# elcritch/figdraw

Hardware: AMD Instinct MI355X
Metric: Mpixels/s composited @3840x2160, 300 SDF rects+shadows; % HBM roofline (higher is better)
Workload: dtype f32 (blur taps: u8 x f16 -> f32 MFMA); 1 GPU; S300@4K: renderlist_100 scene at 3840x2160, 300 shadowed SDF rects + full-frame and 360x240 2-pass Gaussian backdrop blur(18) (BASELINE.json configs[2]); draws=707, phases=3, blur_nodes=2, fragments=41088819, parallelism=single GPU, frames_in_flight_per_gpu=4, walk_pool_threads=7, walk_pool_threads_default=7

## Files before the change

### figdraw_amd/context.py

```python
from __future__ import annotations

import ctypes as C
import os
import subprocess
from typing import Optional

import numpy as np

from . import scene as S

_HERE = os.path.dirname(os.path.abspath(__file__))
LIB_PATH = os.path.join(_HERE, "libfigdraw_hip.so")
_lib = None

_F4 = C.c_float * 4
_F2 = C.c_float * 2
_COL4 = S.CColor * 4


class FigdrawHipError(RuntimeError):
    def __init__(self, code: int, msg: str):
        super().__init__(f"[{code}] {msg}")
        self.code = code

# ... 90 lines not shown
    if hasattr(L, "fdh_put_glyph_outlines"):
        L.fdh_put_glyph_outlines.argtypes = [vp, vp, C.c_int, C.c_uint32, vp]
        L.fdh_glyph_batch_stats.argtypes = [vp, C.POINTER(GlyphBatchStats)]
        L.fdh_sizeof_glyph_outline.argtypes = []
    if hasattr(L, "fdh_put_glyph_outline_cubic"):
        L.fdh_put_glyph_outline_cubic.argtypes = [vp, C.c_int64, C.c_int, C.c_int, vp, C.c_int, C.c_uint32, C.c_int * 4]
    if hasattr(L, "fdh_put_glyph_coverage_batch"):
        L.fdh_put_glyph_coverage_batch.argtypes = [vp, vp, C.c_int, C.c_uint32, vp]
        L.fdh_glyph_coverage_batch_stats.argtypes = [vp, C.POINTER(GlyphBatchStats)]
    if hasattr(L, "fdh_put_glyph_outlines_cubic"):
        L.fdh_put_glyph_outlines_cubic.argtypes = [vp, vp, C.c_int, C.c_uint32, vp]
        L.fdh_put_glyph_coverage_batch_cubic.argtypes = [vp, vp, C.c_int, C.c_uint32, vp]
    L.fdh_read_pixels.argtypes = [vp, C.c_int, C.c_int, C.c_int, C.c_int, vp]
    L.fdh_debug_read_surface.argtypes = [vp, C.c_int, vp]
    L.fdh_scene_retain.argtypes = [vp, vp, C.c_float, C.c_float, C.c_int, _F4]
    L.fdh_scene_update_nodes.argtypes = [vp, C.c_int, C.c_int, C.c_int, vp, vp]
    L.fdh_scene_replace_root.argtypes = [vp, C.c_int, C.c_int, vp, C.c_int, vp]
    L.fdh_scene_insert_root.argtypes = [vp, C.c_int, C.c_int, vp, C.c_int, vp]
    L.fdh_scene_render.argtypes = [vp]
    L.fdh_scene_stats.argtypes = [vp, C.POINTER(C.c_int64), C.POINTER(C.c_int64)]
    L.fdh_debug_record_digest.argtypes = [vp, C.POINTER(C.c_uint64)]
    L.fdh_debug_verify_upload.argtypes = [vp, C.POINTER(C.c_uint32)]
    L.fdh_debug_bin_digest.argtypes = [vp, C.POINTER(C.c_uint64)]
    L.fdh_debug_staging_store_bytes.argtypes = [C.c_int, C.POINTER(C.c_int64)]
    L.fdh_last_upload_bytes.argtypes = [vp, C.POINTER(C.c_int64)]
    L.fdh_record_begin.argtypes = [vp]
    L.fdh_record_json.argtypes = [vp]
    L.fdh_record_json.restype = C.c_char_p
    L.fdh_frame_device_ptr.argtypes = [vp, C.POINTER(vp), C.POINTER(C.c_int), C.POINTER(C.c_int), C.POINTER(C.c_int64)]
    L.fdh_sync.argtypes = [vp]
    L.fdh_flush.argtypes = [vp]
    L.fdh_set_ui_scale.argtypes = [vp, C.c_float]
    L.fdh_render_frame.argtypes = [vp, vp, C.c_float, C.c_float, C.c_int, _F4]
    L.fdh_set_stripe.argtypes = [vp, C.c_int, C.c_int]
    L.fdh_set_blur_route.argtypes = [vp, C.c_int]
    L.fdh_set_cull.argtypes = [vp, C.c_int]
    L.fdh_culled_draws.argtypes = [vp, C.POINTER(C.c_int64)]
    L.fdh_set_walk_threads.argtypes = [vp, C.c_int]
    L.fdh_debug_host_times.argtypes = [vp, C.POINTER(C.c_int64)]
    L.fdh_walk_stats.argtypes = [vp, C.POINTER(C.c_int), C.POINTER(C.c_int64)]
    L.fdh_stripe_rows.argtypes = [C.c_int, C.c_int, C.c_int, C.POINTER(C.c_int), C.POINTER(C.c_int)]
    L.fdh_comm_unique_id.argtypes = [C.c_char_p]
    L.fdh_comm_init.argtypes = [vp, C.c_char_p, C.c_int, C.c_int]
    L.fdh_comm_destroy.argtypes = [vp]
    L.fdh_comm_share.argtypes = [vp, vp]
    L.fdh_gather_stripes.argtypes = [vp, C.c_int, vp]
# ... 363 lines not shown
    def scene_render(self):
        self._ck(self.L.fdh_scene_render(self.h))

    def scene_stats(self):
        a, b = C.c_int64(), C.c_int64()
        self._ck(self.L.fdh_scene_stats(self.h, C.byref(a), C.byref(b)))
        return a.value, b.value

    def last_upload_bytes(self) -> int:
        out = C.c_int64()
        self._ck(self.L.fdh_last_upload_bytes(self.h, C.byref(out)))
        return out.value

    def verify_upload(self):
        out = (C.c_uint32 * 24)()
        self._ck(self.L.fdh_debug_verify_upload(self.h, out))
        return list(out)

    def bin_digest(self):
        out = (C.c_uint64 * 8)()
        self._ck(self.L.fdh_debug_bin_digest(self.h, out))
        return list(out)[:5]

    def record_digest(self) -> int:
        out = C.c_uint64()
        self._ck(self.L.fdh_debug_record_digest(self.h, C.byref(out)))
        return out.value

    def replay_calls(self, calls):
        for call in calls:
            name, args = call[0], call[1:]
            if name == "begin_frame":
                self.begin_frame(self.W, self.H, *args)
            else:
                getattr(self, name)(*args)

    def set_stripe(self, y0: int, y1: int):
        self._ck(self.L.fdh_set_stripe(self.h, int(y0), int(y1)))

    def set_cull(self, mode: int):
        self._ck(self.L.fdh_set_cull(self.h, int(mode)))

    def set_walk_threads(self, n: int):
        self._ck(self.L.fdh_set_walk_threads(self.h, int(n)))

    def host_times(self):
# ... 218 lines not shown
```

### figdraw_amd/csrc/fdh_capi.cpp

```cpp
#include <string>

#include "fdh_context.h"
#include "fdh_damage.h"
#include "../../include/figdraw_hip_damage.h"
#include "../../include/figdraw_hip_pick.h"
#include "../../include/figdraw_hip_readback.h"
#include "../../include/figdraw_hip_stream.h"
#include "../../include/figdraw_hip_exact.h"
#include "../../include_glyphs/figdraw_hip_glyphs.h"
#include "../../include_glyphs/figdraw_hip_coverage.h"
#include "../../include_glyphs/figdraw_hip_cubic.h"

using fdh::Context;

namespace {
thread_local std::string g_last_error;

template <typename F>
int guard(F&& f) {
  try {
    f();
    return FDH_OK;
  } catch (const fdh::Error& e) {
    g_last_error = e.what();
// ... 11 lines not shown
  return reinterpret_cast<Context*>(c);
}
}

extern "C" {

const char* fdh_last_error(void) { return g_last_error.c_str(); }
#if FDH_STATS
extern "C++" { namespace fdh { void debug_counters(unsigned long long out[128], bool reset); void debug_wave_times(unsigned long long* out); } }
__attribute__((visibility("default"))) int fdh_debug_wave_times(unsigned long long* out) { fdh::debug_wave_times(out); return 0; }
__attribute__((visibility("default"))) int fdh_debug_counters(unsigned long long out[128], int reset) { fdh::debug_counters(out, reset != 0); return 0; }
#endif
int fdh_saturated_core(const float rect[4], const float rx[4], const float ry[4], int mode, float factor, float spread,
                       const float shape[2], float aa, int out_px[4]) {
  return guard([&] { fdh::saturated_core_of(rect, rx, ry, mode, factor, spread, shape, aa, out_px); });
}
__attribute__((visibility("default"))) int fdh_saturated_core_union(const float rect[4], const float rx[4], const float ry[4], int mode, float factor, float spread,
                             const float shape[2], float aa, int push, int out_px[12], int* n_out) {
  return guard([&] {
    if (!out_px || !n_out) throw fdh::Error(FDH_ERR_INVALID, "fdh_saturated_core_union: null pointer");
    *n_out = fdh::saturated_core_union_of(rect, rx, ry, mode, factor, spread, shape, aa, push, out_px);
  });
}
int fdh_blur_weight_fragments(float blur_radius, int vertical, float* dense, uint16_t* frag_bits, int* reach, int* k_steps) {
  return guard([&] {
    if (!dense || !frag_bits || !reach || !k_steps) throw fdh::Error(FDH_ERR_INVALID, "fdh_blur_weight_fragments: null pointer");
    fdh::blur_weight_fragments(blur_radius, vertical != 0, dense, frag_bits, reach, k_steps);
  });
}
const char* fdh_version(void) { return "figdraw_hip 0.1.0 (gfx950)"; }
int fdh_sizeof_fig(void) { return (int)sizeof(FdhFig); }
int fdh_sizeof_glyph(void) { return (int)sizeof(FdhGlyph); }
int fdh_sizeof_draw_op(void) { return (int)sizeof(FdhDrawOp); }
int fdh_sizeof_text_rect(void) { return (int)sizeof(FdhTextRect); }

int fdh_create(FdhContext** out, int atlas_size, float pixel_scale, int device, uint32_t flags) {
  return guard([&] {
    if (!out) throw fdh::Error(FDH_ERR_INVALID, "fdh_create: null out pointer");
    *out = nullptr;
    *out = reinterpret_cast<FdhContext*>(new Context(atlas_size, pixel_scale, device, flags));
  });
}
int fdh_destroy(FdhContext* c) { return guard([&] { delete C(c); }); }
int fdh_set_stream(FdhContext* c, void* s) { return guard([&] { C(c)->set_stream(s); }); }

int fdh_begin_frame(FdhContext* c, int w, int h, int clear, const float rgba[4]) {
// ... 323 lines not shown
```

### figdraw_amd/csrc/fdh_context.h

```cpp
#pragma once
#include <hip/hip_runtime.h>

#include <algorithm>
#include <atomic>
#include <chrono>
#include <condition_variable>
#include <cstdint>
#include <cstdlib>
#include <cstring>
#include <exception>
#include <memory>
#include <mutex>
#include <stdexcept>
#include <string>
#include <thread>
#include <unordered_map>
#include <vector>

#include "../../include/figdraw_hip.h"
#include "../../include/figdraw_hip_pick.h"
#include "../../include/figdraw_hip_readback.h"
#include "../../include/figdraw_hip_stream.h"
#include "fdh_kernels.h"
#include "fdh_plain.h"
// ... 122 lines not shown
  void reset_atlas(int minimum_size) { sync(); atlas_.reset(minimum_size, stream_); }
  int atlas_size() const { return atlas_.size(); }
  int64_t atlas_packed_area() const { return atlas_.packed_area(); }

  void read_pixels(int x, int y, int w, int h, uint8_t* out);
  void frame_device_ptr(void** p, int* w, int* h, int64_t* pitch_bytes);
  void debug_read_surface(int which, uint8_t* out);
  void record_begin();
  const char* record_json();
  void sync();
  void set_stream(void* s);

  void set_ui_scale(float s) { ui_scale_ = s; }
  float ui_scale() const { return ui_scale_; }
  void render_frame(const FdhScene* scene, float fw, float fh, bool clear, const float rgba[4]);
  void scene_retain(const FdhScene* scene, float fw, float fh, bool clear, const float rgba[4]) { retained_.retain(scene, fw, fh, clear, rgba); scene_render(); }
  void scene_update_nodes(int layer, int first, int count, const FdhFig* nodes, const FdhScene* side) { retained_.update_nodes(layer, first, count, nodes, side); }
  void scene_replace_root(int layer, int slot, const FdhFig* subtree, int n, const FdhScene* side, bool insert) { retained_.replace_root(layer, slot, subtree, n, side, insert); }
  void scene_render();
  void scene_stats(int64_t* walked, int64_t* reused) const { retained_.stats(walked, reused); }
  int64_t uploaded_bytes() { drain(); return uploaded_bytes_; }
  void debug_verify_upload(uint32_t out[24]);
  void debug_bin_digest(uint64_t out[8]);
  uint64_t record_digest();

  void comm_init(const uint8_t id[FDH_COMM_ID_BYTES], int rank, int world);
  void comm_share(Context* owner);
  void comm_destroy();
  void gather_stripes(int dst_rank, void* dst_image);
  void gather_frames(int dst_rank, void* const* dst_images);
  int comm_world() const { return comm_ ? comm_world_ : 1; }

  void set_stripe(int y0, int y1) {
    drain();
    if (damage_.on && y1 > y0) throw Error(FDH_ERR_INVALID, "fdh_set_stripe: damage tracking is on (fdh_set_damage_tracking: not under row stripes)");
    if (readback_.on && y1 > y0) throw Error(FDH_ERR_INVALID, "fdh_set_stripe: damage readback is on (fdh_set_damage_readback: not under row stripes)");
    stripe_y0_ = y0; stripe_y1_ = y1;
  }
  void set_damage_tracking(bool on);
  void damage_bins(uint8_t* mask, int cap, int* bins_x, int* bins_y, int* n_damaged, bool changed_only);
  void set_damage_readback(bool on);
  void read_damage(const FdhDamageTile** tiles, const uint8_t** pixels, int* n_tiles, int* frame_w, int* frame_h, int* full);
  void read_damage_into(uint8_t* image, int64_t pitch_bytes, int w, int h, int* n_tiles);
  void read_damage_coded(const FdhCodedTile** tiles, const uint8_t** payload, int* n_tiles, int64_t* payload_bytes, int* frame_w, int* frame_h, int* full);
  void set_damage_exact(bool on);
  void damage_exact_stats(int* n_pending, int* n_changed, int* fresh);
// ... 227 lines not shown
```

### figdraw_amd/csrc/fdh_debug.cpp

```cpp
#include "fdh_context.h"

#include <cstring>

namespace fdh {

uint64_t Context::record_digest() {
  drain();
  uint64_t h = 1469598103934665603ull;
  auto mix = [&](const void* p, size_t n) { const uint8_t* b = static_cast<const uint8_t*>(p); for (size_t i = 0; i < n; i++) { h ^= b[i]; h *= 1099511628211ull; } };
  const uint64_t n = n_total_;
  mix(&n, sizeof n);
  uint32_t ext_base = 0;
  for (const Piece& p : pieces_) {
    const Lane& L = lane(p.lane);
    for (uint32_t i = 0; i < p.n; i++) {
      DrawRec r = L.recs[p.first + i];
      record_host_form(r);
      if (r.op_mode & F_GENERAL) r.ext = r.ext - p.ext_first + ext_base;
      mix(&r, sizeof r);
    }
    ext_base += p.n_ext;
  }
  for (const Piece& p : pieces_) { const Lane& L = lane(p.lane); for (uint32_t i = 0; i < p.n; i++) mix(&L.bins[p.first + i].box, sizeof(BBox)); }
  for (const Piece& p : pieces_) { const Lane& L = lane(p.lane); for (uint32_t i = 0; i < p.n_ext; i++) mix(&L.exts[p.ext_first + i], sizeof(QuadExt)); }
// ... 85 lines not shown
  std::vector<uint2> lists(np * nb * stride);
  FDH_HIP(hipMemcpy(counts.data(), J.counts, counts.size() * 4, hipMemcpyDeviceToHost));
  FDH_HIP(hipMemcpy(lists.data(), J.lists, lists.size() * sizeof(uint2), hipMemcpyDeviceToHost));
  uint64_t h = 1469598103934665603ull;
  auto mix = [&](uint32_t v) { for (int k = 0; k < 4; k++) { h ^= (v >> (8 * k)) & 255u; h *= 1099511628211ull; } };
  for (size_t p = 0; p < np; p++) {
    const Phase& ph = J.phases[p];
    const bool whole = p == 0;
    for (int by = 0; by < J.bins_y; by++)
      for (int bx = 0; bx < J.bins_x; bx++) {
        if (!whole && (bx < ph.bin_x0 || bx >= ph.bin_x1 || by < ph.bin_y0 || by >= ph.bin_y1)) continue;
        const size_t b = p * nb + (size_t)by * J.bins_x + bx;
        const uint32_t c = counts[b];
        mix(c);
        out[1] += c;
        if (c == 0) out[2]++;
        if (c > stride) { out[4]++; continue; }
        for (uint32_t e = 0; e < c; e++) { const uint2 v = lists[b * stride + e]; mix(v.x); mix(v.y); if (v.x == 0) out[3]++; }
      }
  }
  out[0] = h;
}

void Context::debug_read_surface(int which, uint8_t* out) {
  need_device("debug_read_surface");
  drain();
  if (which == 4) {
    FDH_HIP(hipSetDevice(device_));
    FDH_HIP(hipStreamSynchronize(stream_));
    FDH_HIP(hipMemcpy(out, atlas_.level0(), (size_t)atlas_.size() * atlas_.size() * 4, hipMemcpyDeviceToHost));
    return;
  }
  const uint32_t* src = which == 0 ? fb_ : which == 1 ? blur_tmp_ : which == 2 ? backdrop_ : which == 3 ? dbg_snap_ : nullptr;
  if (!src) throw Error(FDH_ERR_INVALID, "debug_read_surface: no such surface (or no frame yet)");
  FDH_HIP(hipSetDevice(device_));
  FDH_HIP(hipStreamSynchronize(stream_));
  FDH_HIP(hipMemcpy(out, src, (size_t)W_ * H_ * 4, hipMemcpyDeviceToHost));
}

}
```

### figdraw_amd/csrc/fdh_record.cpp

```cpp
#include <algorithm>
#include <cmath>
#include <cstdio>
#include <cstring>

#include "fdh_context.h"
#include "fdh_host.h"

namespace fdh {

void Recorder::shrink_to_ink(const AtlasEntry& e, bool use_alpha, int level_t) {
  static const bool enabled = [] { const char* v = std::getenv("FDH_INK_BOUNDS"); return !v || std::atoi(v) != 0; }();
  if (!enabled || !e.has_ink || level_t < 0 || lane_->recs.empty()) return;
  DrawRec& r = lane_->recs.back();
  BBox& b = lane_->bins.back().box;
  if ((r.op_mode & F_GENERAL) || b.x1 <= b.x0 || b.y1 <= b.y0) return;
  const InkBox ib = (use_alpha ? e.ink_a : e.ink_rgb)[std::min(level_t / 16, kInkLevels - 1)];
  if (ib.x1 <= ib.x0 || ib.y1 <= ib.y0) { b = BBox{0, 0, 0, 0}; r.bx0 = r.by0 = r.bx1 = r.by1 = 0; return; }
  const double S = (double)cx_->atlas_.size();
  auto range = [&](double ua, double ut, double o, double inv, double lo_t, double hi_t, int& p0, int& p1) {
    const double A = (ut - ua) * inv * S, B = ua * S - 0.5 - A * o;
    if (!(std::fabs(A) > 1e-12)) return;
    double c0 = ((lo_t - 3.0) - B) / A, c1 = ((hi_t + 2.0) - B) / A;
    if (c0 > c1) std::swap(c0, c1);
    if (!(c0 > -1.0e6 && c1 < 1.0e6)) return;
// ... 118 lines not shown
  flags |= BR_HAS_CORE | (rot ? BR_GENERAL : 0u);
  if (op == OP_DRAW && (mode == 9u || mode == 11u || mode == 12u)) {
    flags |= BR_CORE_REMOVED;
    if (!rot && (om & F_SOLID) && fill_mode == 0u && mode != 11u) flags |= ((mode == 9u ? 3u : 4u) + ell) << LE_PATH_SHIFT;
  } else {
    if (op == OP_DRAW && (om & F_SOLID) && fill_mode == 0u && mode != 17u) {
      flags |= LE_PLAIN;
      const uint32_t code = mode == 3u ? 1u : mode == 7u ? 2u : 0u;
      if (code && !rot) flags |= (code + ell) << LE_PATH_SHIFT;
    }
    if (op == OP_DRAW && mode == 3u) {
      uint32_t a = r.col[0] & r.col[1] & r.col[2] & r.col[3];
      if (fill_mode != 0u) a &= r.mid & r.stop;
      if ((a >> 24) == 255u) flags |= LE_OPAQUE;
    }
  }
  return flags;
}
static inline bool colour_as_floats(uint32_t om) {
  const uint32_t mode = om & 255u;
  const bool atlas_mode = mode == 0u || (mode >= 13u && mode <= 16u);
  return !(((om & F_GENERAL) && !(om & F_EDGE32)) || atlas_mode || mode >= 18u || ((om >> 12) & 15u) != OP_DRAW || !(om & F_SOLID));
}
void record_host_form(DrawRec& r) {
  if (colour_as_floats(r.op_mode)) r.col[1] = r.col[2] = r.col[3] = r.col[0];
}

void Recorder::link_share(uint32_t idx) {
  if ((int)idx <= phase_floor_) return;
  const DrawRec& b = lane_->recs[idx];
  BinRec& pa = lane_->bins[idx - 1];
  const uint32_t code = (pa.flags >> LE_PATH_SHIFT) & 15u;
  if (code == 0u) return;
  const DrawRec& r = lane_->recs[idx - 1];
  const uint32_t om = r.op_mode, mode = om & 255u;
  if (mode == 7u) return;
  const uint32_t omb = b.op_mode, modeb = omb & 255u;
  const bool simple_b = ((omb >> 12) & 15u) == OP_DRAW && !(omb & F_GENERAL) && (omb & F_SOLID) && ((omb >> 9) & 7u) == 0u &&
                        (modeb == 3u || modeb == 9u || modeb == 12u) && ((omb ^ om) & F_ELLIP) == 0u;
  if (simple_b && std::memcmp(&r.ox, &b.ox, 6 * sizeof(float)) == 0 && std::memcmp(r.r, b.r, sizeof r.r) == 0 &&
      std::memcmp(&r.bx0, &b.bx0, 4 * sizeof(int16_t)) == 0 && r.aa == b.aa) {
    const float sax = mode == 9u ? r.p0 : r.p2, say = mode == 9u ? r.p1 : r.p3, sbx = modeb == 9u ? b.p0 : b.p2, sby = modeb == 9u ? b.p1 : b.p3;
    if (sax == sbx && say == sby) pa.flags |= LE_SHARE;
  }
}

void Recorder::commit_bins(uint32_t idx) {
  DrawRec& r = lane_->recs[idx];
// ... 114 lines not shown
  const uint32_t mode = r.op_mode & 255u, op = (r.op_mode >> 12) & 15u;
  const uint32_t fill_mode = (r.op_mode >> 9) & 7u;
  if (!(op == OP_DRAW || op == OP_MASK_PUSH) || !(r.aa > 0.0f)) return false;
  double e;
  if (op == OP_MASK_PUSH || mode == FDH_SDF_CLIP_AA || mode == FDH_SDF_BACKDROP_BLUR) e = 0.5 / r.aa;
  else if (mode == FDH_SDF_DROP_SHADOW) e = std::max(0.0, -(double)(fill_mode == 0u ? r.f1 : 0.0f));
  else if (mode == FDH_SDF_ANNULAR || mode == FDH_SDF_ANNULAR_AA) e = std::max(0.0, (double)r.f0) + 0.5 / r.aa;
  else if (mode == FDH_SDF_INSET_SHADOW && op == OP_DRAW) {
    const double sigma = std::max(0.5 * (double)r.f0, 0.5);
    e = std::max(0.0, 3.7 * sigma + (double)(fill_mode == 0u ? r.f1 : 0.0f));
  } else return false;
  const bool inset = mode == FDH_SDF_INSET_SHADOW;
  const double qhx = r.p0, qhy = r.p1, bx = inset ? qhx : (double)r.p2, by = inset ? qhy : (double)r.p3;
  if (!(qhx > 0.0 && qhy > 0.0 && bx > 0.0 && by > 0.0)) return false;
  double crx[4], cry[4];
  for (int k = 0; k < 4; k++) {
    const double sel = r.r[k];
    if (!(r.op_mode & F_ELLIP)) { crx[k] = cry[k] = std::max(sel, 0.0); continue; }
    if (sel < 0.0) { crx[k] = cry[k] = -sel - 1.0; continue; }
    const double pv = std::floor(sel + 0.5), hi = std::floor(pv / 4096.0);
    crx[k] = (pv - 4096.0 * hi) * bx / 4095.0;
    cry[k] = hi * by / 4095.0;
  }
  enum { TR = 0, BR = 1, TL = 2, BL = 3 };
  LocalRect &H = out[1], &V = out[2];
  H.xl = -(bx - e); H.xr = bx - e;
  V.yb = -(by - e); V.yt = by - e;
  if (!(r.op_mode & F_ELLIP)) {
    const double k = 0.2929;
    auto rr = [&](int i) { return std::max(crx[i] - e, 0.0); };
    const double mr = std::max(rr(TR), rr(BR)), ml = std::max(rr(TL), rr(BL)), mt = std::max(rr(TR), rr(TL)), mb = std::max(rr(BR), rr(BL));
    out[0].xr = (bx - e) - k * mr;
    out[0].xl = -(bx - e) + k * ml;
    out[0].yt = (by - e) - k * mt;
    out[0].yb = -(by - e) + k * mb;
    H.yt = (by - e) - mt; H.yb = -(by - e) + mb;
    V.xr = (bx - e) - mr; V.xl = -(bx - e) + ml;
  } else {
    H.yt = std::min(by - e, by - std::max(cry[TR], cry[TL])); H.yb = -std::min(by - e, by - std::max(cry[BR], cry[BL]));
    V.xr = std::min(bx - e, bx - std::max(crx[TR], crx[BR])); V.xl = -std::min(bx - e, bx - std::max(crx[TL], crx[BL]));
    const double ah = std::max(H.xr - H.xl, 0.0) * std::max(H.yt - H.yb, 0.0), av = std::max(V.xr - V.xl, 0.0) * std::max(V.yt - V.yb, 0.0);
    out[0] = ah >= av ? H : V;
  }
  if (inset)
    for (int k = 0; k < 3; k++) { out[k].xl += r.p2; out[k].xr += r.p2; out[k].yb -= r.p3; out[k].yt -= r.p3; }
  return true;
}
static bool core_pixels(const DrawRec& r, float w_px, float h_px, const LocalRect& c, int16_t px[4]) {
  if (!c.ok()) return false;
  const double qhx = r.p0, qhy = r.p1;
#ifndef FDH_CORE_SLACK
#define FDH_CORE_SLACK (1.0 / 16.0)
#endif
  const double slack = FDH_CORE_SLACK;
  const double cxl = r.ox + w_px * (c.xl / (2.0 * qhx) + 0.5) + slack, cxr = r.ox + w_px * (c.xr / (2.0 * qhx) + 0.5) - slack;
  const double cyt = r.oy + h_px * (0.5 - c.yt / (2.0 * qhy)) + slack, cyb = r.oy + h_px * (0.5 - c.yb / (2.0 * qhy)) - slack;
  double ix0 = std::ceil(cxl - 0.5), ix1 = std::floor(cxr - 0.5) + 1.0, iy0 = std::ceil(cyt - 0.5), iy1 = std::floor(cyb - 0.5) + 1.0;
  ix0 = std::max(ix0, (double)r.ox); ix1 = std::min(ix1, (double)r.ox + w_px);
  iy0 = std::max(iy0, (double)r.oy); iy1 = std::min(iy1, (double)r.oy + h_px);
  auto c16 = [](double v) { return (int16_t)std::min(std::max(v, -32768.0), 32767.0); };
  if (!(ix1 > ix0 && iy1 > iy0)) return false;
  px[0] = c16(ix0); px[1] = c16(iy0); px[2] = c16(ix1); px[3] = c16(iy1);
  return true;
}
static bool core_union_on() {
  static const bool enabled = [] { const char* v = std::getenv("FDH_CORE_UNION"); return !v || std::atoi(v) != 0; }();
// ... 89 lines not shown
  const float* py = q.py;
  BBox b = q.b;
  bands_ = CoreBands{};
  const bool cullable = ((r.op_mode >> 12) & 15u) == OP_DRAW && culling();
  const float fields[] = {r.p0, r.p1, r.p2, r.p3, r.f0, r.f1, r.r[0], r.r[1], r.r[2], r.r[3], r.aa, r.aux, r.aux2};
  bool params_finite = true;
  for (const float v : fields) params_finite = params_finite && std::isfinite(v);
  if (!q.finite || !params_finite) {
    if (cullable) { FDH_CULLED(); return false; }
    r.bx0 = r.by0 = r.bx1 = r.by1 = 0; push_rec(b); return true;
  }
  if (cullable && !bbox_visible(b)) { FDH_CULLED(); return false; }
  r.bx0 = b.x0; r.by0 = b.y0; r.bx1 = b.x1; r.by1 = b.y1;
  const bool aligned = px[3] == px[0] && px[2] == px[1] && py[3] == py[2] && py[0] == py[1] && px[1] > px[0] && py[0] > py[3];
  const bool bezier = (r.op_mode & 255u) >= 18u && (r.op_mode & 255u) <= 20u;
  if (aligned) {
    r.ox = px[3];
    r.oy = py[3];
    r.inv_w = 1.0f / (px[1] - px[0]);
    r.inv_h = 1.0f / (py[0] - py[3]);
    r.kx = 2.0f * r.p0 * r.inv_w;
    r.ky = 2.0f * r.p1 * r.inv_h;
    if (!bezier) bands_ = set_saturated_core(r, px[1] - px[0], py[0] - py[3]);
  }
  if (!aligned || bezier) {
    QuadExt& q = *lane_->exts.slot();
    std::memset(static_cast<void*>(&q), 0, sizeof q);
    static const int TRI[2][3] = {{3, 0, 1}, {2, 3, 1}};
    const uint32_t mode = r.op_mode & 255u;
    const bool atlas_mode = mode == 0u || (mode >= 13u && mode <= 16u);
    const float uax = atlas_mode ? r.r[0] : 0.0f, uay = atlas_mode ? r.r[1] : 0.0f, utx = atlas_mode ? r.r[2] : 1.0f, uty = atlas_mode ? r.r[3] : 1.0f;
    const float vu[4] = {uax, utx, utx, uax}, vv[4] = {uty, uty, uay, uay};
    bool edge32 = true;
    const long long xm = 2LL * cx_->W_ + 129, ym = 2LL * cx_->H_ + 129;
    for (int t = 0; t < 2; t++) {
      long long X[3], Y[3];
      for (int k = 0; k < 3; k++) { X[k] = 2 * (long long)px[TRI[t][k]]; Y[k] = 2 * (long long)py[TRI[t][k]]; }
      long long area2 = (X[1] - X[0]) * (Y[2] - Y[0]) - (Y[1] - Y[0]) * (X[2] - X[0]);
      const long long sgn = area2 >= 0 ? 1 : -1;
      for (int k = 0; k < 3; k++) {
        const int i0 = (k + 1) % 3, i1 = (k + 2) % 3;
        long long A = -(Y[i1] - Y[i0]) * sgn, B = (X[i1] - X[i0]) * sgn;
        long long C = -(B * Y[i0]) - (A * X[i0]);
        q.e[t][k].a = (int32_t)A; q.e[t][k].b = (int32_t)B; q.e[t][k].c = C;
        {
          const long long aa = A < 0 ? -A : A, ab = B < 0 ? -B : B, ac = C < 0 ? -(C + 1) : C;
// ... 610 lines not shown
```

### figdraw_amd/csrc/fdh_types.h

```cpp
#pragma once
#include <stdint.h>

#ifndef FDH_MX_LO
#define FDH_MX_LO 0
#endif

namespace fdh {

constexpr int kTile = 8;
constexpr int kTileW = 4 * kTile;
constexpr int kTileH = kTile;
constexpr int kWavesPerWg = 4;
constexpr int kWgW = kTileW;
constexpr int kWgH = kTileH * kWavesPerWg;
constexpr int kBin = 64;
constexpr int kWgsPerBin = (kBin / kWgW) * (kBin / kWgH);
constexpr int kMaskDepth = 16;
constexpr int kDeepMinDefault = 24;
constexpr int kDeepMinInFlight = 40;
constexpr int kDeepStripMinDefault = 16;
constexpr int kMaxMips = 14;
constexpr int kMaxBlurTaps = 36;

enum : uint32_t { OP_DRAW = 0, OP_MASK_PUSH = 1, OP_MASK_POP = 2, OP_RMASK_BEGIN = 3, OP_RMASK_END = 4 };
// ... 6 lines not shown
constexpr uint32_t F_TEXEL_1TO1 = 1u << 20;
constexpr uint32_t F_EDGE32 = 1u << 21;

struct alignas(16) DrawRec {
  uint32_t op_mode;
  uint32_t ext;
  float ox, oy;
  float inv_w, inv_h;
  float p0, p1;
  float p2, p3;
  float f0, f1;
  float r[4];
  uint32_t col[4];
  uint32_t mid, stop;
  float aa;
  float aux;
  float aux2;
  int16_t bx0, by0, bx1, by1;
  int16_t ix0, iy0, ix1, iy1;
  float kx, ky;
  uint32_t _pad;
};
static_assert(sizeof(DrawRec) == 128, "DrawRec must be 128 bytes");

struct alignas(16) QuadExt {
  struct Edge { int32_t a, b; int64_t c; };
  Edge e[2][3];
  float inv_sum[2];
  uint32_t own;
  float fw_u[2], fw_v[2];
  float lod[2];
  float _pad[3];
  float core[4];
  float lm[2][6];
};
static_assert(sizeof(QuadExt) == 208 && offsetof(QuadExt, core) == 144 && offsetof(QuadExt, lm) == 160, "QuadExt: 208 bytes, core at 144, lm at 160");

struct alignas(8) BBox { int16_t x0, y0, x1, y1; };

struct alignas(8) BinRec { BBox box; int16_t ix0, iy0, ix1, iy1; uint32_t flags; uint32_t grow; uint16_t hy0, hy1, vx0, vx1; };
static_assert(sizeof(BinRec) == 32, "BinRec must be 32 bytes");
constexpr uint32_t BR_HAS_CORE = 1u, BR_CORE_REMOVED = 2u;
constexpr uint32_t BR_GENERAL = 4u;
constexpr uint32_t BR_CURVE = 8u;
constexpr uint32_t BR_BOX_EXACT = 16u;
constexpr uint32_t LE_PLAIN = 1u << 31;
// ... 33 lines not shown
```

### figdraw_amd/csrc/k_composite.hip

```cpp
#include "fdh_device.h"
#include "fdh_shade.h"
#include "fdh_damage.h"

#ifndef FDH_TU
#define FDH_TU 0
#endif

namespace fdh {

__device__ __forceinline__ void order_bins_wave(const uint32_t* __restrict__ counts, int* __restrict__ order, int nx, int nb, uint32_t* offs, int lane, int cls,
                                                int deep_min = 0, uint32_t* __restrict__ deep_out = nullptr) {
#pragma unroll
  for (int k = 0; k < 4; k++) offs[lane + 64 * k] = 0;
  __builtin_amdgcn_wave_barrier();
  constexpr int kU = 8;
  const int nc = (nb - cls + 7) >> 3;
  for (int i0 = lane; i0 < nc; i0 += 64 * kU) {
    uint32_t c[kU];
#pragma unroll
    for (int k = 0; k < kU; k++) c[k] = i0 + 64 * k < nc ? counts[cls + 8 * (i0 + 64 * k)] : 0xffffffffu;
#pragma unroll
    for (int k = 0; k < kU; k++) if (c[k] != 0xffffffffu) atomicAdd(&offs[255u - min(c[k], 255u)], 1u);
  }
  __builtin_amdgcn_wave_barrier();
// ... 9 lines not shown
    __builtin_amdgcn_wave_barrier();
    offs[4 * lane] = base; offs[4 * lane + 1] = base + a; offs[4 * lane + 2] = base + a + b; offs[4 * lane + 3] = base + a + b + c2;
  }
  __builtin_amdgcn_wave_barrier();
  if (deep_out != nullptr && lane == 0) {
    const int m = min(max(deep_min, 1), 255);
    __hip_atomic_store(deep_out + cls, offs[256 - m], __ATOMIC_RELAXED, __HIP_MEMORY_SCOPE_SYSTEM);
  }
  __builtin_amdgcn_wave_barrier();
  for (int i0 = lane; i0 < nc; i0 += 64 * kU) {
    uint32_t c[kU];
#pragma unroll
    for (int k = 0; k < kU; k++) c[k] = i0 + 64 * k < nc ? counts[cls + 8 * (i0 + 64 * k)] : 0xffffffffu;
#pragma unroll
    for (int k = 0; k < kU; k++)
      if (c[k] != 0xffffffffu) {
        const int i = cls + 8 * (i0 + 64 * k), row = i / nx;
        order[8 * (int)atomicAdd(&offs[255u - min(c[k], 255u)], 1u) + cls] = (row << 16) | (i - row * nx);
      }
  }
}

struct Corner { float rx, ry; bool same; };
__device__ __forceinline__ Corner pick_corner(bool ellip, float px, float py, float bx, float by, float r0, float r1, float r2, float r3) {
  const float sel = (px > 0.0f) ? ((py > 0.0f) ? r0 : r1) : ((py > 0.0f) ? r2 : r3);
  Corner c;
  if (!ellip) { c.rx = sel; c.ry = sel; c.same = true; return c; }
  const float pv = __builtin_floorf(sel + 0.5f);
  const float hi = __builtin_floorf(pv * (1.0f / 4096.0f));
  float rx = (pv - 4096.0f * hi) * bx * (1.0f / 4095.0f);
  float ry = hi * by * (1.0f / 4095.0f);
  const bool circle = sel < 0.0f;
  const float rc = -sel - 1.0f;
  rx = circle ? rc : rx;
  ry = circle ? rc : ry;
  const bool zero = rx <= 0.0f || ry <= 0.0f;
  c.rx = zero ? 0.0f : rx;
  c.ry = zero ? 0.0f : ry;
  c.same = c.rx == c.ry;
  return c;
}
__device__ __forceinline__ float sd_ellipse_nb(float px, float py, float rx, float ry) {
  const float sx = __builtin_fmaxf(rx, 0.000001f), sy = __builtin_fmaxf(ry, 0.000001f);
  const float isx = frcp(sx), isy = frcp(sy);
  const float ax = px * isx, ay = py * isy;
  const float k0 = fsqrt(ax * ax + ay * ay);
  const float bx = ax * isx, by = ay * isy;
  const float k1 = fsqrt(bx * bx + by * by);
  const float d = k0 * (k0 - 1.0f) * frcp(__builtin_fmaxf(k1, 0.000001f));
  const float inner = -__builtin_fminf(sx, sy);
  return k0 <= 0.000001f ? inner : d;
}
template <int N, bool kPerY>
__device__ __forceinline__ void shape_distNy(bool ellip, const float* px, const float* pyv, float bx, float by, float r0, float r1, float r2,
                                             float r3, float* out) {
  Corner c[N];
  float qx[N], qy[N];
  bool need = false, diag = false;
#pragma unroll
  for (int k = 0; k < N; k++) {
    const float py = pyv[kPerY ? k : 0];
    c[k] = pick_corner(ellip, px[k], py, bx, by, r0, r1, r2, r3);
    qx[k] = __builtin_fabsf(px[k]) - bx + c[k].rx;
    qy[k] = __builtin_fabsf(py) - by + c[k].ry;
// ... 2 lines not shown
    need = need || (!c[k].same && corner);
  }
  const bool any_diag = __any(diag);
#pragma unroll
  for (int k = 0; k < N; k++) {
    float m = __builtin_fmaxf(qx[k], qy[k]);
    if (any_diag) {
      const float e = fsqrt(qx[k] * qx[k] + qy[k] * qy[k]);
      m = (qx[k] > 0.0f && qy[k] > 0.0f) ? e : m;
    }
    out[k] = m - c[k].rx;
  }
  if (!ellip) return;
  const bool any_ellipse = __any(need);
#pragma unroll
  for (int k = 0; k < N; k++) {
    const bool corner = qx[k] > 0.0f && qy[k] > 0.0f;
    float de = __builtin_fmaxf(qx[k] - c[k].rx, qy[k] - c[k].ry);
    if (any_ellipse) {
      const float e = sd_ellipse_nb(qx[k], qy[k], c[k].rx, c[k].ry);
      de = corner ? e : de;
    }
    out[k] = c[k].same ? out[k] : de;
  }
}
template <int N>
__device__ __forceinline__ void shape_distN(bool ellip, const float* px, float py, float bx, float by, float r0, float r1, float r2,
                                            float r3, float* out) {
  shape_distNy<N, false>(ellip, px, &py, bx, by, r0, r1, r2, r3, out);
}

constexpr int kFastWaves = 5;
constexpr int kAtlasWaves = 5;
constexpr int kSlowWaves = 4;
constexpr int kSlowAtlasWaves = 3;
constexpr int kRotWaves = 4;
constexpr int kUniformWaves = 6;
constexpr int kWinCols = 64, kWinRows = 12, kWinStride = 68;
constexpr int kDeepSlots = 6;
constexpr int kDeepSlotFloats = 16 * 64;
constexpr int kDeepHdr = 8;
[[maybe_unused]] constexpr int kDeepLdsDwords = kDeepSlots * (kDeepSlotFloats + kDeepHdr) + kDeepSlots + 2;
constexpr uint32_t DT_NOP = 0, DT_PACKED = 1, DT_PACKED_BLACK = 2, DT_GENERIC = 3, DT_SELF17 = 4, DT_UNIFORM_PRE = 5;
struct DeepRing {
  float* data;
  uint32_t* hdr;
// ... 262 lines not shown
```

### figdraw_amd/csrc/k_composite_strip.inc

```
  static_assert(kRole == 0 || (kPaths == 4 && kFull), "deep strips: the no-clip build's full-frame launch only");
  constexpr int kStripsPerBin = kWgsPerBin * kWavesPerWg;
  constexpr int mslot = 0;
  constexpr bool kBlender = kRole == 1, kShader = kRole == 2;
  constexpr bool kOpaque = (kPaths & 32) != 0;
  static_assert(!kOpaque || (kPaths == (4 | 32) && kRole == 0), "the opaque form exists for the no-clip build only");
  using FT = std::conditional_t<kOpaque, F4o, F4>;
  uint32_t (*mask_stack)[kMaskDepth][64] = reinterpret_cast<uint32_t (*)[kMaskDepth][64]>(composite_lds);
  const DeepRing ring(composite_lds);
  uint32_t rank = 0, unit = 0;
  const int tx1 = tx0 + kTileW, ty1 = ty0 + kTileH;
  const int px0 = tx0 + (lane & 7) * 4, py = ty0 + (lane >> 3);
  const size_t spill_at = ((size_t)bin * kStripsPerBin + (size_t)sidx) * 64 + (size_t)lane;
  auto stack_put = [&](const int depth, const uint32_t v) __attribute__((always_inline)) {
    if (depth < kMaskDepth) mask_stack[mslot][depth][lane] = v;
    else __hip_atomic_store(P.mask_spill + (size_t)(depth - kMaskDepth) * P.spill_stride + spill_at, v, __ATOMIC_RELAXED, __HIP_MEMORY_SCOPE_AGENT);
  };
  auto stack_get = [&](const int depth) __attribute__((always_inline)) -> uint32_t {
    if (depth < kMaskDepth) return mask_stack[mslot][depth][lane];
    return __hip_atomic_load(P.mask_spill + (size_t)(depth - kMaskDepth) * P.spill_stride + spill_at, __ATOMIC_RELAXED, __HIP_MEMORY_SCOPE_AGENT);
  };
  constexpr bool kMasks = (kPaths & 4) == 0;
#if FDH_TIMING
  const unsigned long long T0 = FDH_NOW(), W0 = wall_clock64();
  unsigned long long T_cull = 0, T_rec = 0, T_shade = 0, T_cnt = 0, n_draws_t = 0, T_cull_core = 0, n_core_t = 0, n_all_t = 0;
// ... 125 lines not shown
    if (m == 0) continue;
    const unsigned long long m_plainc = m_core & __ballot((int32_t)idx < 0);
    u32x4 plain_col = {0u, 0u, 0u, 0u};
    if (kBlender) plain_col = *reinterpret_cast<const u32x4*>(draws[idx & LE_INDEX].col);
    const uint32_t code_l = idx & (15u << LE_PATH_SHIFT);
    const unsigned long long m_simple = m & ~m_core & __ballot((kPaths & 3) == 0 ? code_l != 0u : (code_l - 1u) < (4u << LE_PATH_SHIFT));
    auto dist4 = [&](const DrawRec& r, const f2 pxa, const f2 pxb, const float py_, const float bx, const float by, f2& da, f2& db) __attribute__((always_inline)) {
      const bool top = py_ > 0.0f;
      const float rR = top ? r.r[0] : r.r[1], rL = top ? r.r[2] : r.r[3];
      const float ay = __builtin_fabsf(py_) - by;
      const f2 rra = {pxa.x > 0.0f ? rR : rL, pxa.y > 0.0f ? rR : rL}, rrb = {pxb.x > 0.0f ? rR : rL, pxb.y > 0.0f ? rR : rL};
      const f2 axa = {__builtin_fabsf(pxa.x), __builtin_fabsf(pxa.y)}, axb = {__builtin_fabsf(pxb.x), __builtin_fabsf(pxb.y)};
      const f2 qxa = axa - bx + rra, qxb = axb - bx + rrb;
      const f2 qya = ay + rra, qyb = ay + rrb;
      f2 ma = {__builtin_fmaxf(qxa.x, qya.x), __builtin_fmaxf(qxa.y, qya.y)}, mb = {__builtin_fmaxf(qxb.x, qyb.x), __builtin_fmaxf(qxb.y, qyb.y)};
      const f2 lowa = {__builtin_fminf(qxa.x, qya.x), __builtin_fminf(qxa.y, qya.y)}, lowb = {__builtin_fminf(qxb.x, qyb.x), __builtin_fminf(qxb.y, qyb.y)};
      if (__any(lowa.x > 0.0f || lowa.y > 0.0f || lowb.x > 0.0f || lowb.y > 0.0f)) {
        const f2 sa2 = qxa * qxa + qya * qya, sb2 = qxb * qxb + qyb * qyb;
        ma.x = lowa.x > 0.0f ? fsqrt(sa2.x) : ma.x; ma.y = lowa.y > 0.0f ? fsqrt(sa2.y) : ma.y;
        mb.x = lowb.x > 0.0f ? fsqrt(sb2.x) : mb.x; mb.y = lowb.y > 0.0f ? fsqrt(sb2.y) : mb.y;
      }
      da = ma - rra; db = mb - rrb;
    };
    auto dist4e = [&](const DrawRec& r, const f2 pxa, const f2 pxb, const float py_, const float bx, const float by, f2& oa, f2& ob) __attribute__((always_inline)) {
      const float px4[4] = {pxa.x, pxa.y, pxb.x, pxb.y};
      float d4[4];
      shape_distN<4>(true, px4, py_, bx, by, r.r[0], r.r[1], r.r[2], r.r[3], d4);
      oa = {d4[0], d4[1]}; ob = {d4[2], d4[3]};
    };
    auto edge_geom = [&](const DrawRec& r, const bool inset, const bool ellip, f2& lxa, f2& lxb, float& pyy, f2& da, f2& db) __attribute__((always_inline)) {
      const float shx = inset ? r.p0 : r.p2, shy = inset ? r.p1 : r.p3;
      pyy = local_y_up(r, cy);
      float lx4[4];
      local_x4(r, cx0, lx4);
      lxa = {lx4[0], lx4[1]}; lxb = {lx4[2], lx4[3]};
      if ((kPaths & 3) == 0 && ellip) dist4e(r, lxa, lxb, pyy, shx, shy, da, db); else dist4(r, lxa, lxb, pyy, shx, shy, da, db);
    };
    auto edge_blend = [&](const DrawRec& r, const uint32_t mode, const bool ellip, const bool inq, const float m_p2, const float m_p3, const float m_f0, const float m_f1,
                          const u32x4 m_col, const f2 lxa, const f2 lxb, const float pyy, const f2 da, const f2 db, FT& A0, FT& A1, FT& A2, FT& A3, const uint32_t rk) __attribute__((always_inline)) {
      f2 ala, alb;
      if (mode == 3u) {
        ala = {cover_aa(da.x, r.aa), cover_aa(da.y, r.aa)}; alb = {cover_aa(db.x, r.aa), cover_aa(db.y, r.aa)};
      } else if (mode == 12u) {
        const float h = m_f0 * 0.5f;
        const f2 ea = da + h, eb = db + h;
        const f2 ga = {__builtin_fabsf(ea.x), __builtin_fabsf(ea.y)}, gb = {__builtin_fabsf(eb.x), __builtin_fabsf(eb.y)};
        ala = {cover_aa(ga.x - h, r.aa), cover_aa(ga.y - h, r.aa)}; alb = {cover_aa(gb.x - h, r.aa), cover_aa(gb.y - h, r.aa)};
        if (__all(ala.x == 0.0f && ala.y == 0.0f && alb.x == 0.0f && alb.y == 0.0f)) {
          if (kShader) deep_nop(rk);
          return;
        }
      } else if (mode == 9u) {
        f2 sha, shb;
        if ((kPaths & 3) == 0 && ellip) dist4e(r, lxa - m_p2, lxb - m_p2, pyy + m_p3, r.p0, r.p1, sha, shb); else dist4(r, lxa - m_p2, lxb - m_p2, pyy + m_p3, r.p0, r.p1, sha, shb);
        const float spread = m_f1;
        const f2 sda = sha + spread, sdb = shb + spread;
        const float rs = frcp(__builtin_fmaxf(0.5f * m_f0, 0.5f));
        const f2 za = f2{__builtin_fminf(sda.x, 0.0f), __builtin_fminf(sda.y, 0.0f)} * rs, zb = f2{__builtin_fminf(sdb.x, 0.0f), __builtin_fminf(sdb.y, 0.0f)} * rs;
// ... 1111 lines not shown
```

Before: 193,700 Mpixels/s.

## Precompute per-rect quadrant centre to pick a single corner radius per strip

The host stores the rect's pixel centre in the DrawRec padding field. The strip kernel uses it to check whether a whole tile lies in one quadrant, and if so takes a single corner radius, skipping the per-pixel corner select and the vector radius arithmetic in the SDF distance. The change also widens the saturated-core rects of drop shadows by the shadow grow amount, so more tiles count as fully covered. It adds a margin test per strip, a debug counter API and an env toggle. There is some risk of precision or coverage mismatch near the centre lines and at the grown core edges.

```diff
diff --git a/figdraw_amd/context.py b/figdraw_amd/context.py
--- a/figdraw_amd/context.py
+++ b/figdraw_amd/context.py
@@ -136,6 +136,8 @@
     L.fdh_debug_record_digest.argtypes = [vp, C.POINTER(C.c_uint64)]
     L.fdh_debug_verify_upload.argtypes = [vp, C.POINTER(C.c_uint32)]
     L.fdh_debug_bin_digest.argtypes = [vp, C.POINTER(C.c_uint64)]
+    if hasattr(L, "fdh_debug_quadrant_strips"):
+        L.fdh_debug_quadrant_strips.argtypes = [vp, C.POINTER(C.c_uint64)]
     L.fdh_debug_staging_store_bytes.argtypes = [C.c_int, C.POINTER(C.c_int64)]
     L.fdh_last_upload_bytes.argtypes = [vp, C.POINTER(C.c_int64)]
     L.fdh_record_begin.argtypes = [vp]
@@ -545,6 +547,11 @@
         self._ck(self.L.fdh_debug_bin_digest(self.h, out))
         return list(out)[:5]
 
+    def quadrant_strips(self):
+        out = (C.c_uint64 * 4)()
+        self._ck(self.L.fdh_debug_quadrant_strips(self.h, out))
+        return tuple(int(v) for v in out)
+
     def record_digest(self) -> int:
         out = C.c_uint64()
         self._ck(self.L.fdh_debug_record_digest(self.h, C.byref(out)))
diff --git a/figdraw_amd/csrc/fdh_capi.cpp b/figdraw_amd/csrc/fdh_capi.cpp
--- a/figdraw_amd/csrc/fdh_capi.cpp
+++ b/figdraw_amd/csrc/fdh_capi.cpp
@@ -57,6 +57,19 @@
     *n_out = fdh::saturated_core_union_of(rect, rx, ry, mode, factor, spread, shape, aa, push, out_px);
   });
 }
+__attribute__((visibility("default"))) int fdh_quadrant_centre(float ox, float oy, float w_px, float h_px, float kx, float ky, int* cxp, int* cyp) {
+  return guard([&] {
+    if (!cxp || !cyp) throw fdh::Error(FDH_ERR_INVALID, "fdh_quadrant_centre: null pointer");
+    const uint32_t v = fdh::quadrant_centre(ox, oy, w_px, h_px, kx, ky);
+    *cxp = (int)(int16_t)(v & 0xffffu); *cyp = (int)(int16_t)(v >> 16);
+  });
+}
+__attribute__((visibility("default"))) int fdh_debug_quadrant_strips(FdhContext* c, uint64_t out[4]) {
+  return guard([&] {
+    if (!out) throw fdh::Error(FDH_ERR_INVALID, "fdh_debug_quadrant_strips: null pointer");
+    C(c)->debug_quadrant_strips(out);
+  });
+}
 int fdh_blur_weight_fragments(float blur_radius, int vertical, float* dense, uint16_t* frag_bits, int* reach, int* k_steps) {
   return guard([&] {
     if (!dense || !frag_bits || !reach || !k_steps) throw fdh::Error(FDH_ERR_INVALID, "fdh_blur_weight_fragments: null pointer");
diff --git a/figdraw_amd/csrc/fdh_context.h b/figdraw_amd/csrc/fdh_context.h
--- a/figdraw_amd/csrc/fdh_context.h
+++ b/figdraw_amd/csrc/fdh_context.h
@@ -168,6 +168,7 @@
   int64_t uploaded_bytes() { drain(); return uploaded_bytes_; }
   void debug_verify_upload(uint32_t out[24]);
   void debug_bin_digest(uint64_t out[8]);
+  void debug_quadrant_strips(uint64_t out[4]);
   uint64_t record_digest();
 
   void comm_init(const uint8_t id[FDH_COMM_ID_BYTES], int rank, int world);
diff --git a/figdraw_amd/csrc/fdh_debug.cpp b/figdraw_amd/csrc/fdh_debug.cpp
--- a/figdraw_amd/csrc/fdh_debug.cpp
+++ b/figdraw_amd/csrc/fdh_debug.cpp
@@ -131,6 +131,31 @@
   out[0] = h;
 }
 
+void Context::debug_quadrant_strips(uint64_t out[4]) {
+  drain();
+  for (int i = 0; i < 4; i++) out[i] = 0;
+  for (const Piece& p : pieces_) {
+    const Lane& L = lane(p.lane);
+    for (uint32_t i = 0; i < p.n; i++) {
+      const DrawRec& r = L.recs[p.first + i];
+      const BinRec& br = L.bins[p.first + i];
+      if (((br.flags >> LE_PATH_SHIFT) & 15u) == 0u || bbox_empty(br.box)) continue;
+      out[0]++;
+      if (r._pad != kQuadrantNone) out[1]++;
+      int core[12];
+      binrec_core_rects(br, core);
+      for (int ty = br.box.y0 / kTileH * kTileH; ty < br.box.y1; ty += kTileH)
+        for (int tx = br.box.x0 / kTileW * kTileW; tx < br.box.x1; tx += kTileW) {
+          bool in_core = false;
+          for (int k = 0; k < 3; k++) in_core = in_core || (tx >= core[4 * k] && ty >= core[4 * k + 1] && tx + kTileW <= core[4 * k + 2] && ty + kTileH <= core[4 * k + 3]);
+          if (in_core) continue;
+          out[2]++;
+          if (strip_quadrant(r._pad, tx, ty) >= 0) out[3]++;
+        }
+    }
+  }
+}
+
 void Context::debug_read_surface(int which, uint8_t* out) {
   need_device("debug_read_surface");
   drain();
diff --git a/figdraw_amd/csrc/fdh_record.cpp b/figdraw_amd/csrc/fdh_record.cpp
--- a/figdraw_amd/csrc/fdh_record.cpp
+++ b/figdraw_amd/csrc/fdh_record.cpp
@@ -164,8 +164,18 @@
   const bool atlas_mode = mode == 0u || (mode >= 13u && mode <= 16u);
   return !(((om & F_GENERAL) && !(om & F_EDGE32)) || atlas_mode || mode >= 18u || ((om >> 12) & 15u) != OP_DRAW || !(om & F_SOLID));
 }
+static inline bool has_quadrant_field(uint32_t om) {
+  const uint32_t mode = om & 255u, op = (om >> 12) & 15u;
+  const bool atlas_mode = mode == 0u || (mode >= 13u && mode <= 16u);
+  return !(om & F_GENERAL) && !atlas_mode && mode < 18u && (op == OP_DRAW || op == OP_MASK_PUSH);
+}
+static bool quadrant_on() {
+  static const bool enabled = [] { const char* v = std::getenv("FDH_QUADRANT"); return !v || std::atoi(v) != 0; }();
+  return enabled;
+}
 void record_host_form(DrawRec& r) {
   if (colour_as_floats(r.op_mode)) r.col[1] = r.col[2] = r.col[3] = r.col[0];
+  if (has_quadrant_field(r.op_mode)) r._pad = 0u;
 }
 
 void Recorder::link_share(uint32_t idx) {
@@ -326,6 +336,7 @@
     crx[k] = (pv - 4096.0 * hi) * bx / 4095.0;
     cry[k] = hi * by / 4095.0;
   }
+  const double grow = mode == FDH_SDF_DROP_SHADOW && op == OP_DRAW && fill_mode == 0u && r.f1 > 0.0f ? (double)r.f1 : 0.0;
   enum { TR = 0, BR = 1, TL = 2, BL = 3 };
   LocalRect &H = out[1], &V = out[2];
   H.xl = -(bx - e); H.xr = bx - e;
@@ -346,6 +357,7 @@
     const double ah = std::max(H.xr - H.xl, 0.0) * std::max(H.yt - H.yb, 0.0), av = std::max(V.xr - V.xl, 0.0) * std::max(V.yt - V.yb, 0.0);
     out[0] = ah >= av ? H : V;
   }
+  if (grow > 0.0) { H.xl -= grow; H.xr += grow; V.yb -= grow; V.yt += grow; }
   if (inset)
     for (int k = 0; k < 3; k++) { out[k].xl += r.p2; out[k].xr += r.p2; out[k].yb -= r.p3; out[k].yt -= r.p3; }
   return true;
@@ -481,6 +493,7 @@
     r.kx = 2.0f * r.p0 * r.inv_w;
     r.ky = 2.0f * r.p1 * r.inv_h;
     if (!bezier) bands_ = set_saturated_core(r, px[1] - px[0], py[0] - py[3]);
+    if (has_quadrant_field(r.op_mode)) r._pad = quadrant_on() ? quadrant_centre(r.ox, r.oy, px[1] - px[0], py[0] - py[3], r.kx, r.ky) : kQuadrantNone;
   }
   if (!aligned || bezier) {
     QuadExt& q = *lane_->exts.slot();
diff --git a/figdraw_amd/csrc/fdh_types.h b/figdraw_amd/csrc/fdh_types.h
--- a/figdraw_amd/csrc/fdh_types.h
+++ b/figdraw_amd/csrc/fdh_types.h
@@ -1,4 +1,5 @@
 #pragma once
+#include <stddef.h>
 #include <stdint.h>
 
 #ifndef FDH_MX_LO
@@ -52,6 +53,30 @@
   uint32_t _pad;
 };
 static_assert(sizeof(DrawRec) == 128, "DrawRec must be 128 bytes");
+
+constexpr int16_t kQuadrantUnknown = INT16_MIN;
+constexpr int kQuadrantMargin = 2;
+constexpr uint32_t kQuadrantNone = 0x80008000u;
+#if defined(__HIPCC__)
+#define FDH_HOST_DEVICE __host__ __device__
+#else
+#define FDH_HOST_DEVICE
+#endif
+FDH_HOST_DEVICE inline int strip_quadrant(uint32_t pad, int tx0, int ty0) {
+  const int cxp = (int)(int16_t)(pad & 0xffffu), cyp = (int)(int16_t)(pad >> 16);
+  const bool right = tx0 > cxp + kQuadrantMargin, left = tx0 + kTileW <= cxp - kQuadrantMargin;
+  const bool below = ty0 > cyp + kQuadrantMargin, above = ty0 + kTileH <= cyp - kQuadrantMargin;
+  if (pad == kQuadrantNone || !(right || left) || !(above || below)) return -1;
+  return (right ? 1 : 0) | (above ? 2 : 0);
+}
+inline uint32_t quadrant_centre(float ox, float oy, float w_px, float h_px, float kx, float ky) {
+  const double cx = (double)ox + 0.5 * (double)w_px - 0.5, cy = (double)oy + 0.5 * (double)h_px - 0.5;
+  const double lim = 32000.0;
+  if (!(w_px > 0.0f && h_px > 0.0f && kx >= 1.0f / 64.0f && ky >= 1.0f / 64.0f && cx > -lim && cx < lim && cy > -lim && cy < lim && w_px < 1.0e6f && h_px < 1.0e6f))
+    return kQuadrantNone;
+  const int ix = (int)cx - ((double)(int)cx > cx ? 1 : 0), iy = (int)cy - ((double)(int)cy > cy ? 1 : 0);
+  return (uint32_t)(uint16_t)(int16_t)ix | ((uint32_t)(uint16_t)(int16_t)iy << 16);
+}
 
 struct alignas(16) QuadExt {
   struct Edge { int32_t a, b; int64_t c; };
diff --git a/figdraw_amd/csrc/k_composite.hip b/figdraw_amd/csrc/k_composite.hip
--- a/figdraw_amd/csrc/k_composite.hip
+++ b/figdraw_amd/csrc/k_composite.hip
@@ -55,8 +55,7 @@
 }
 
 struct Corner { float rx, ry; bool same; };
-__device__ __forceinline__ Corner pick_corner(bool ellip, float px, float py, float bx, float by, float r0, float r1, float r2, float r3) {
-  const float sel = (px > 0.0f) ? ((py > 0.0f) ? r0 : r1) : ((py > 0.0f) ? r2 : r3);
+__device__ __forceinline__ Corner decode_corner(bool ellip, float sel, float bx, float by) {
   Corner c;
   if (!ellip) { c.rx = sel; c.ry = sel; c.same = true; return c; }
   const float pv = __builtin_floorf(sel + 0.5f);
@@ -73,6 +72,10 @@
   c.same = c.rx == c.ry;
   return c;
 }
+__device__ __forceinline__ Corner pick_corner(bool ellip, float px, float py, float bx, float by, float r0, float r1, float r2, float r3) {
+  const float sel = (px > 0.0f) ? ((py > 0.0f) ? r0 : r1) : ((py > 0.0f) ? r2 : r3);
+  return decode_corner(ellip, sel, bx, by);
+}
 __device__ __forceinline__ float sd_ellipse_nb(float px, float py, float rx, float ry) {
   const float sx = __builtin_fmaxf(rx, 0.000001f), sy = __builtin_fmaxf(ry, 0.000001f);
   const float isx = frcp(sx), isy = frcp(sy);
@@ -121,6 +124,38 @@
       de = corner ? e : de;
     }
     out[k] = c[k].same ? out[k] : de;
+  }
+}
+__device__ __forceinline__ void shape_dist4_quadrant(const Corner c, const float* px, float py, float bx, float by, float* out) {
+  float qx[4];
+  const float qy = __builtin_fabsf(py) - by + c.ry;
+  bool diag = false;
+#pragma unroll
+  for (int k = 0; k < 4; k++) {
+    qx[k] = __builtin_fabsf(px[k]) - bx + c.rx;
+    diag = diag || (qx[k] > 0.0f && qy > 0.0f);
+  }
+  const bool any_diag = __any(diag);
+  if (c.same) {
+#pragma unroll
+    for (int k = 0; k < 4; k++) {
+      float m = __builtin_fmaxf(qx[k], qy);
+      if (any_diag) {
+        const float e = fsqrt(qx[k] * qx[k] + qy * qy);
+        m = (qx[k] > 0.0f && qy > 0.0f) ? e : m;
+      }
+      out[k] = m - c.rx;
+    }
+    return;
+  }
+#pragma unroll
+  for (int k = 0; k < 4; k++) {
+    float de = __builtin_fmaxf(qx[k] - c.rx, qy - c.ry);
+    if (any_diag) {
+      const float e = sd_ellipse_nb(qx[k], qy, c.rx, c.ry);
+      de = (qx[k] > 0.0f && qy > 0.0f) ? e : de;
+    }
+    out[k] = de;
   }
 }
 template <int N>
diff --git a/figdraw_amd/csrc/k_composite_strip.inc b/figdraw_amd/csrc/k_composite_strip.inc
--- a/figdraw_amd/csrc/k_composite_strip.inc
+++ b/figdraw_amd/csrc/k_composite_strip.inc
@@ -171,10 +171,31 @@
       }
       da = ma - rra; db = mb - rrb;
     };
+    auto dist4q = [&](const float rq, const f2 pxa, const f2 pxb, const float py_, const float bx, const float by, f2& da, f2& db) __attribute__((always_inline)) {
+      const float ay = __builtin_fabsf(py_) - by;
+      const f2 axa = {__builtin_fabsf(pxa.x), __builtin_fabsf(pxa.y)}, axb = {__builtin_fabsf(pxb.x), __builtin_fabsf(pxb.y)};
+      const f2 qxa = axa - bx + rq, qxb = axb - bx + rq;
+      const float qy = ay + rq;
+      f2 ma = {__builtin_fmaxf(qxa.x, qy), __builtin_fmaxf(qxa.y, qy)}, mb = {__builtin_fmaxf(qxb.x, qy), __builtin_fmaxf(qxb.y, qy)};
+      const f2 lowa = {__builtin_fminf(qxa.x, qy), __builtin_fminf(qxa.y, qy)}, lowb = {__builtin_fminf(qxb.x, qy), __builtin_fminf(qxb.y, qy)};
+      if (__any(lowa.x > 0.0f || lowa.y > 0.0f || lowb.x > 0.0f || lowb.y > 0.0f)) {
+        const float qy2 = qy * qy;
+        const f2 sa2 = qxa * qxa + qy2, sb2 = qxb * qxb + qy2;
+        ma.x = lowa.x > 0.0f ? fsqrt(sa2.x) : ma.x; ma.y = lowa.y > 0.0f ? fsqrt(sa2.y) : ma.y;
+        mb.x = lowb.x > 0.0f ? fsqrt(sb2.x) : mb.x; mb.y = lowb.y > 0.0f ? fsqrt(sb2.y) : mb.y;
+      }
+      da = ma - rq; db = mb - rq;
+    };
     auto dist4e = [&](const DrawRec& r, const f2 pxa, const f2 pxb, const float py_, const float bx, const float by, f2& oa, f2& ob) __attribute__((always_inline)) {
       const float px4[4] = {pxa.x, pxa.y, pxb.x, pxb.y};
       float d4[4];
       shape_distN<4>(true, px4, py_, bx, by, r.r[0], r.r[1], r.r[2], r.r[3], d4);
+      oa = {d4[0], d4[1]}; ob = {d4[2], d4[3]};
+    };
+    auto dist4eq = [&](const float sel, const f2 pxa, const f2 pxb, const float py_, const float bx, const float by, f2& oa, f2& ob) __attribute__((always_inline)) {
+      const float px4[4] = {pxa.x, pxa.y, pxb.x, pxb.y};
+      float d4[4];
+      shape_dist4_quadrant(decode_corner(true, sel, bx, by), px4, py_, bx, by, d4);
       oa = {d4[0], d4[1]}; ob = {d4[2], d4[3]};
     };
     auto edge_geom = [&](const DrawRec& r, const bool inset, const bool ellip, f2& lxa, f2& lxb, float& pyy, f2& da, f2& db) __attribute__((always_inline)) {
@@ -183,6 +204,15 @@
       float lx4[4];
       local_x4(r, cx0, lx4);
       lxa = {lx4[0], lx4[1]}; lxb = {lx4[2], lx4[3]};
+      const int quadrant = strip_quadrant(r._pad, tx0, ty0);
+      if (quadrant >= 0) {
+        const bool right = (quadrant & 1) != 0, above = (quadrant & 2) != 0;
+        FDH_COUNT(72);
+        const float rR = above ? r.r[0] : r.r[1], rL = above ? r.r[2] : r.r[3];
+        const float rq = right ? rR : rL;
+        if ((kPaths & 3) == 0 && ellip) dist4eq(rq, lxa, lxb, pyy, shx, shy, da, db); else dist4q(rq, lxa, lxb, pyy, shx, shy, da, db);
+        return;
+      }
       if ((kPaths & 3) == 0 && ellip) dist4e(r, lxa, lxb, pyy, shx, shy, da, db); else dist4(r, lxa, lxb, pyy, shx, shy, da, db);
     };
     auto edge_blend = [&](const DrawRec& r, const uint32_t mode, const bool ellip, const bool inq, const float m_p2, const float m_p3, const float m_f0, const float m_f1,
```

Measured after the change: 194,300 Mpixels/s, median of 6. No clear change (+0.3%).
